# openfheorg/openfhe-development

Hardware: AMD Instinct MI355X
Metric: NTT GB/s vs HBM roofline + CKKS EvalMultKeySwitch/sec, N=2^16 L=30, 1/2/4/8 GPU (higher is better)
Workload: dtype u64; 1 GPU; batched fwd+inv negacyclic NTT, N=2^16, L=30 x 60-bit limbs, 1024 polynomials per GPU (BASELINE configs[1]); global_batch=1024, parallelism=batch-sharded x1, no data-path collective

## Files before the change

openfhe-development_amd/csrc/fhe_hip.cpp:

```cpp
#include "../../include/fhe_hip.h"

#include <algorithm>
#include <cmath>
#include <cstdio>
#include <cstdlib>
#include <map>
#include <mutex>
#include <shared_mutex>
#include <string>
#include <vector>

#include "basis_kernels.h"
#include "bfv_kernels.h"
#include "elemwise_kernels.h"
#include "host_math.h"
#include "ntt_kernels.h"
#include "ntt_static.h"
#include "ntt_row8.h"
#include "rt.h"
#include "sampler_kernels.h"
#include "blake2_kernels.h"

using namespace fhe;

static thread_local std::string g_lastError;
static fhe_status fail(fhe_status code, const std::string& msg) {
    g_lastError = msg;
    return code;
}
#define RT_CHECK(expr)                                                                  \
    do {                                                                                \
        const char* _e = (expr);                                                        \
        if (_e)                                                                         \
            return fail(FHE_ERR_DEVICE, std::string(#expr) + ": " + _e);                \
    } while (0)
#define ARG_CHECK(cond, msg)                  \
    do {                                      \
        if (!(cond))                          \
            return fail(FHE_ERR_ARG, msg);    \
    } while (0)

extern "C" const char* fhe_last_error(void) { return g_lastError.c_str(); }
extern "C" const char* fhe_version(void) {
#ifdef FHE_EMU
    return "fhe_hip 0.1 (TEST lane emulator build — not a product build)";
#else
    return "fhe_hip 0.1 (gfx950)";
#endif
}
extern "C" int fhe_device_count(void) { return rt::device_count(); }

namespace fhe {
namespace host {
bool is_prime(uint64_t n) {
    static const uint64_t w[] = {2, 3, 5, 7, 11, 13, 17, 19, 23, 29, 31, 37};
    if (n < 2)
        return false;
    for (uint64_t p : w) {
        if (n == p)
            return true;
        if (n % p == 0)
            return false;
    }
    uint64_t d = n - 1;
    int s      = 0;
    while (!(d & 1)) {
        d >>= 1;
        ++s;
    }
    for (uint64_t a : w) {
        uint64_t x = powmod(a, d, n);
        if (x == 1 || x == n - 1)
            continue;
        bool comp = true;
        for (int r = 1; r < s && comp; ++r) {
            x = mulmod(x, x, n);
            if (x == n - 1)
                comp = false;
        }
        if (comp)
            return false;
    }
    return true;
}
bool is_primitive_root_2n(uint64_t psi, uint64_t twoN, uint64_t q) {
    return psi != 0 && psi < q && powmod(psi, twoN / 2, q) == q - 1;
}
uint64_t first_prime(uint32_t bits, uint64_t m) {
    uint64_t q = (uint64_t)1 << bits, r = q % m, c = q + 1 - r;
    if (r > 0)
        c += m;
    while (!is_prime(c))
        c += m;
    return c;
}
uint64_t last_prime(uint32_t bits, uint64_t m) {
    uint64_t q = (uint64_t)1 << bits, r = q % m, c = q + 1 - r;
    if (r < 2)
        c -= m;
    while (!is_prime(c))
        c -= m;
// ... 499 lines not shown
    a.canonLevels = 1;
    while ((1u << a.canonLevels) < pp.outBound)
        ++a.canonLevels;
    if (canonOut)
        for (uint32_t i = 0; i < pp.nSteps; ++i)
            if (pp.steps[i].bHi >= pp.steps[i].bLo)
                a.canonStep = i;
    for (uint32_t i = 0; i < 6; ++i)
        a.steps[i] = i < pp.nSteps ? pp.steps[i] : NttStep{0, 0, -1, 0, 0, 0, 0, 0};
    a.sel = sel;
    const uint32_t grid        = tiles_for(c, a.rows);
    const uint32_t tilesPerRow = c->N >= (uint32_t)kTile ? (c->N >> kTileLog) : 1u;
    a.xcdSwizzle = (c->N >= (uint32_t)kTile && ((nLimbs * tilesPerRow) % 8u == 0)) ? 1u : 0u;
    a.epiMode = 0, a.epiSplit = 0, a.epiAStride = 0, a.epiAFirst = 0;
    a.epiA = nullptr, a.epiC = nullptr, a.epiOut0 = a.epiOut1 = nullptr;
    a.proMode = 0, a.proSrcLimb = 0;
    a.inDelta = 0, a.epiADelta = 0;
    return grid;
}
static int static_mode(const fhe_ctx* c, const PassPlan& pp, bool inverse) {
    const bool twoPass = c->logN > (uint32_t)kTileLog;
    const int fclass = pp.inBound <= 1 ? 1 : 9;
    return inverse ? ((pp.layoutA || !twoPass) ? 1 : 0) : fclass;
}
static bool row8_for(uint32_t T) {
    static const int forced = [] {
        const char* v = std::getenv("FHE_NTT_ROW8");
        return v && (v[0] == '0' || v[0] == '1') ? v[0] - '0' : -1;
    }();
    return forced >= 0 ? forced == 1 : T <= 11u;
}
static fhe_status launch_pass(const fhe_ctx* c, const PassPlan& pp, bool inverse, const uint64_t* xin, uint64_t* xout,
                              const LimbSel& sel, uint32_t nLimbs, uint32_t batch, bool canonOut, void* stream,
                              uint32_t inStride = 0, uint32_t inFirst = 0, uint32_t outStride = 0, uint32_t outFirst = 0,
                              const NttEpilogue* epi = nullptr, const uint32_t* proSrcLimb = nullptr, int64_t inDelta = 0) {
    NttPassArgs a;
    const uint32_t grid = fill_pass_args(c, pp, inverse, xin, xout, sel, nLimbs, batch, canonOut, inStride, inFirst, outStride,
                                         outFirst, a);
    if (inDelta) {
        if (c->logN < (uint32_t)kTileLog)
            return fail(FHE_ERR_UNSUPPORTED, "ntt: separately allocated towers need a ring of at least 4096");
        a.inDelta = inDelta;
    }
    if (proSrcLimb) {
        a.proMode = 1, a.proSrcLimb = *proSrcLimb;
        const int mode = static_mode(c, pp, inverse);
        if (pp.layoutA && !inverse && mode == 1 && pp.T == 4)
            FHE_LAUNCH_BARRIER((ntt_static_kernel<true, false, 4, 1, false, true>), grid, stream, a);
        else if (pp.layoutA && !inverse && mode == 1 && pp.T == 5)
            FHE_LAUNCH_BARRIER((ntt_static_kernel<true, false, 5, 1, false, true>), grid, stream, a);
        else
            return fail(FHE_ERR_UNSUPPORTED, "ntt: no prologue kernel for this pass shape");
        LAUNCH_CHECK();
        return FHE_OK;
    }
    if (epi && epi->mode) {
        a.epiMode = epi->mode, a.epiSplit = epi->split, a.epiAStride = epi->aStride, a.epiAFirst = epi->aFirst;
        a.epiA = epi->A, a.epiC = epi->C, a.epiOut0 = epi->out0, a.epiOut1 = epi->out1;
        a.epiADelta = epi->aDelta;
        const int mode = static_mode(c, pp, inverse);
        bool launched  = false;
#define FHE_EPI_CASE(TT, MODE) \
    if (!launched && !pp.layoutA && !inverse && pp.T == TT && mode == MODE) { \
        FHE_LAUNCH_BARRIER((ntt_static_kernel<false, false, TT, MODE, true>), grid, stream, a); \
        launched = true; \
    }
        FHE_EPI_CASE(12, 9) FHE_EPI_CASE(11, 9) FHE_EPI_CASE(10, 9) FHE_EPI_CASE(9, 9) FHE_EPI_CASE(12, 1)
#undef FHE_EPI_CASE
        if (!launched)
            return fail(FHE_ERR_UNSUPPORTED, "ntt: no epilogue kernel for this pass shape");
        LAUNCH_CHECK();
        return FHE_OK;
    }
    if (c->logN >= (uint32_t)kTileLog) {
        const int mode = static_mode(c, pp, inverse);
        bool launched  = false;
#define FHE_STATIC_CASE(LA, INV, TT, MODE) \
    if (!launched && pp.layoutA == LA && inverse == INV && pp.T == TT && mode == MODE) { \
        FHE_LAUNCH_BARRIER((ntt_static_kernel<LA, INV, TT, MODE>), grid, stream, a); \
        launched = true; \
    }
        if (!pp.layoutA && c->logN > (uint32_t)kTileLog && row8_for(pp.T)) {
            const uint32_t rgrid = a.rows << (c->logN - pp.T);
            a.xcdSwizzle         = ((nLimbs << (c->logN - pp.T)) % 8u == 0) ? 1u : 0u;
#define FHE_ROW8_CASE(INV, TT, MODE) \
    if (!launched && inverse == INV && pp.T == TT && mode == MODE) { \
        FHE_LAUNCH_BARRIER_N((r8::ntt_row8_kernel<INV, TT - 9, MODE>), rgrid, 64u << (TT - 9), stream, a); \
        launched = true; \
    }
            FHE_ROW8_CASE(false, 12, 9) FHE_ROW8_CASE(true, 12, 0) FHE_ROW8_CASE(false, 11, 9) FHE_ROW8_CASE(true, 11, 0)
            FHE_ROW8_CASE(false, 10, 9) FHE_ROW8_CASE(true, 10, 0) FHE_ROW8_CASE(false, 9, 9) FHE_ROW8_CASE(true, 9, 0)
#undef FHE_ROW8_CASE
        }
        FHE_STATIC_CASE(true, false, 4, 1) FHE_STATIC_CASE(true, true, 4, 1)
        FHE_STATIC_CASE(true, false, 5, 1) FHE_STATIC_CASE(true, true, 5, 1)
        FHE_STATIC_CASE(false, false, 12, 9) FHE_STATIC_CASE(false, true, 12, 0)
        FHE_STATIC_CASE(false, false, 11, 9) FHE_STATIC_CASE(false, true, 11, 0)
        FHE_STATIC_CASE(false, false, 10, 9) FHE_STATIC_CASE(false, true, 10, 0)
        FHE_STATIC_CASE(false, false, 9, 9) FHE_STATIC_CASE(false, true, 9, 0)
        FHE_STATIC_CASE(false, false, 12, 1) FHE_STATIC_CASE(false, true, 12, 1)
#undef FHE_STATIC_CASE
        if (!launched)
            return fail(FHE_ERR_UNSUPPORTED, "ntt: no kernel instance for this pass shape");
        LAUNCH_CHECK();
        return FHE_OK;
    }
    if (pp.layoutA) {
        if (inverse)
            FHE_LAUNCH_BARRIER((ntt_pass_kernel<true, true>), grid, stream, a);
        else
            FHE_LAUNCH_BARRIER((ntt_pass_kernel<true, false>), grid, stream, a);
    }
    else {
        if (inverse)
            FHE_LAUNCH_BARRIER((ntt_pass_kernel<false, true>), grid, stream, a);
        else
            FHE_LAUNCH_BARRIER((ntt_pass_kernel<false, false>), grid, stream, a);
    }
    LAUNCH_CHECK();
    return FHE_OK;
}

static uint32_t env_u32(const char* name, uint32_t dflt) {
    const char* v = std::getenv(name);
    return v ? (uint32_t)std::strtoul(v, nullptr, 10) : dflt;
}
static uint32_t ntt_t1(uint32_t logN) {
    const uint32_t dflt = std::max(4u, logN - (uint32_t)kTileLog);
    static const uint32_t forced = env_u32("FHE_NTT_T1", 0);
    if (forced >= 4 && forced <= 5 && logN > (uint32_t)kTileLog && logN - forced >= 9 && logN - forced <= 12)
        return forced;
    return dflt;
}

static bool ntt_epilogue_supported(const fhe_ctx* c) {
    if (c->logN < (uint32_t)kTileLog)
        return false;
    if (c->logN == (uint32_t)kTileLog)
        return true;
    const uint32_t t1 = ntt_t1(c->logN), t2 = c->logN - t1;
    return t2 == 12u || (t1 == 4u && t2 >= 9u && t2 <= 12u);
}
static bool ntt_prologue_supported(const fhe_ctx* c) {
    return c->logN > (uint32_t)kTileLog && ntt_t1(c->logN) <= 5u;
}
static fhe_status ntt_run(fhe_ctx* c, bool inverse, const uint64_t* xin, uint64_t* xout, const uint32_t* limbIdx,
                          uint32_t nLimbs, uint32_t batch, void* stream, uint32_t inStride = 0, uint32_t inFirst = 0,
                          uint32_t outStride = 0, uint32_t outFirst = 0, const NttEpilogue* epi = nullptr,
                          bool canonOut = true, const uint32_t* proSrcLimb = nullptr, int64_t inDelta = 0) {
    ARG_CHECK(c && xin && xout, "fhe_ntt: null argument");
    ARG_CHECK(batch >= 1, "fhe_ntt: batch must be >= 1");
    LimbSel sel;
    if (fhe_status s = make_sel(c, limbIdx, nLimbs, &sel, "fhe_ntt"))
        return s;
    RT_CHECK(rt::set_device(c->device));
    const uint32_t logN = c->logN;
    if (logN <= (uint32_t)kTileLog) {
        PassPlan p;
        plan_pass(inverse, false, logN, logN, &p);
        uint32_t bound = 1;
        mark_uniform(p, logN);
        if (!inverse)
            schedule_fwd(p, logN, &bound);
        p.outBound = bound;
        return launch_pass(c, p, inverse, xin, xout, sel, nLimbs, batch, canonOut, stream, inStride, inFirst, outStride, outFirst, epi,
                           nullptr, inDelta);
    }
    const uint32_t T1 = ntt_t1(logN), T2 = logN - T1;
    PassPlan pa, pb;
    plan_pass(inverse, true, logN, T1, &pa);
// ... 1065 lines not shown
    ARG_CHECK(p && devB && devA && out, "fhe_ks_key_wrap: null argument");
    fhe_ks_key* k = new fhe_ks_key;
    k->plan       = p;
    k->words      = (size_t)p->numPartQ * (p->sizeQ + p->sizeP) << p->ctx->logN;
    k->d_b        = devB;
    k->d_a        = devA;
    k->owned      = false;
    *out          = k;
    return FHE_OK;
}
extern "C" void fhe_ks_key_destroy(fhe_ks_key* k) {
    if (!k)
        return;
    if (k->owned && k->d_b)
        rt::dfree(k->d_b);
    if (k->owned && k->d_a)
        rt::dfree(k->d_a);
    delete k;
}
extern "C" uint64_t* fhe_ks_key_devptr(fhe_ks_key* k, int which) { return k ? (which ? k->d_a : k->d_b) : nullptr; }
extern "C" size_t fhe_ks_key_words(const fhe_ks_key* k) { return k ? k->words : 0; }

struct KsLayout {
    size_t coef = 0, e0 = 0, e1 = 0, md = 0, pcoef = 0, d2 = 0, k0 = 0, k1 = 0, total = 0;
    std::vector<size_t> dig;
};
static KsLayout ks_layout(const fhe_ks_plan* p, uint32_t sizeQl, uint32_t batch) {
    KsLayout w;
    const size_t N = (size_t)1 << p->ctx->logN;
    const uint32_t numParts = std::min((sizeQl + p->alpha - 1) / p->alpha, p->numPartQ);
    w.dig.assign(numParts, 0);
    size_t off = 0;
    w.coef = off, off += (size_t)batch * sizeQl * N;
    for (uint32_t j = 0; j < numParts; ++j) {
        const uint32_t start = p->alpha * j;
        const uint32_t sz    = (j == numParts - 1) ? sizeQl - start : p->alpha;
        w.dig[j] = off, off += (size_t)batch * (sizeQl - sz + p->sizeP) * N;
    }
    w.e0 = off, off += (size_t)batch * (sizeQl + p->sizeP) * N;
    w.e1 = off, off += (size_t)batch * (sizeQl + p->sizeP) * N;
    w.md = off, off += (size_t)2 * batch * sizeQl * N;
    w.pcoef = off, off += (size_t)2 * batch * p->sizeP * N;
    w.d2 = off, off += (size_t)batch * sizeQl * N;
    w.k0 = off, off += (size_t)batch * sizeQl * N;
    w.k1 = off, off += (size_t)batch * sizeQl * N;
    w.total = off;
    return w;
}
extern "C" size_t fhe_ks_workspace_bytes(const fhe_ks_plan* p, uint32_t sizeQl, uint32_t batch) {
    if (!p || sizeQl < 1 || sizeQl > p->sizeQ || batch < 1)
        return 0;
    return ks_layout(p, sizeQl, batch).total * 8;
}

static fhe_status mod_down_core(fhe_ks_plan* p, fhe_ks_plan::Level* lv, const uint64_t* x, uint32_t nTow, uint64_t* pcoef,
                                uint64_t* md, void* st, fhe_conv* down = nullptr, const NttEpilogue* epi = nullptr) {
    fhe_ctx* c            = p->ctx;
    const uint32_t sizeQl = lv->sizeQl, sizeP = p->sizeP, sizeQlP = sizeQl + sizeP;
    std::vector<uint32_t> pIdx(sizeP);
    for (uint32_t j = 0; j < sizeP; ++j)
        pIdx[j] = p->sizeQ + j;
    if (fhe_status s = ntt_run(c, true, x, pcoef, pIdx.data(), sizeP, nTow, st, sizeQlP, sizeQl))
        return s;
    if (fhe_status s = fhe_approx_switch_basis(down ? down : lv->down, pcoef, sizeP, 0, md, sizeQl, 0, nTow, st))
        return s;
    return ntt_run(c, false, md, md, nullptr, sizeQl, nTow, st, 0, 0, 0, 0, epi);
}
static fhe_status mod_down_tail(fhe_ks_plan* p, fhe_ks_plan::Level* lv, const uint64_t* x, const uint64_t* md, uint32_t nTow,
                                uint64_t* out, bool accumulate, void* st) {
    const uint32_t sizeQl = lv->sizeQl, sizeQlP = sizeQl + p->sizeP;
    if (accumulate)
        return elem_run<OP_SUB_MUL_CONST_ACC>(p->ctx, out, x, md, lv->d_PInv, nullptr, sizeQl, nTow, st, "fhe_approx_mod_down",
                                              sizeQlP, 0);
    return elem_run<OP_SUB_MUL_CONST>(p->ctx, out, x, md, lv->d_PInv, nullptr, sizeQl, nTow, st, "fhe_approx_mod_down", sizeQlP, 0);
}
static fhe_status mod_down_run(fhe_ks_plan* p, fhe_ks_plan::Level* lv, const uint64_t* x, uint32_t nTow, uint64_t* out,
                               uint64_t* pcoef, uint64_t* md, void* st) {
    if (fhe_status s = mod_down_core(p, lv, x, nTow, pcoef, md, st))
        return s;
    return mod_down_tail(p, lv, x, md, nTow, out, false, st);
}

static fhe_status ks_precompute_run(fhe_ks_plan* p, fhe_ks_plan::Level* lv, const uint64_t* cin, uint32_t batch,
                                    uint64_t* ws, const KsLayout& w, void* st) {
    fhe_ctx* c            = p->ctx;
    const uint32_t sizeQl = lv->sizeQl;
    if (fhe_status s = fhe_ntt_inv_oop(c, cin, ws + w.coef, nullptr, sizeQl, batch, st))
        return s;
    for (uint32_t j = 0; j < lv->numParts; ++j) {
        const uint32_t nc = (uint32_t)lv->cidx[j].size();
        uint64_t* dj      = ws + w.dig[j];
        if (fhe_status s = fhe_approx_switch_basis(lv->up[j], ws + w.coef, sizeQl, p->alpha * j, dj, nc, 0, batch, st))
            return s;
        if (fhe_status s = ntt_run(c, false, dj, dj, lv->cidx[j].data(), nc, batch, st, 0, 0, 0, 0, nullptr, false))
            return s;
    }
    return FHE_OK;
}
static fhe_status ks_inner_multi_launch(fhe_ks_plan* p, fhe_ks_plan::Level* lv, const fhe_ks_key* const* keys, uint32_t nKeys,
                                        const uint64_t* cin, uint32_t batch, uint64_t* const* e0, uint64_t* const* e1,
                                        const uint64_t* first, const TwPair* dP, uint64_t* ws, const KsLayout& w, void* st,
                                        uint32_t towOff = 0) {
    fhe_ctx* c            = p->ctx;
    const uint32_t sizeQl = lv->sizeQl, sizeP = p->sizeP, sizeQlP = sizeQl + sizeP;
    const uint32_t tilesPerRow = c->N >= (uint32_t)kTile ? (c->N >> kTileLog) : 1u;
    for (uint32_t t0 = 0; t0 < nKeys; t0 += (uint32_t)kMaxMultiKeys) {
        KsInnerMultiArgs g;
        const uint32_t nt = std::min<uint32_t>(kMaxMultiKeys, nKeys - t0);
        for (uint32_t j = 0; j < (uint32_t)kMaxDigits; ++j) {
            g.nc[j]     = j < lv->numParts ? (uint32_t)lv->cidx[j].size() : 0u;
            g.digits[j] = j < lv->numParts ? ws + w.dig[j] + (((size_t)towOff * g.nc[j]) << c->logN) : nullptr;
        }
        for (uint32_t t = 0; t < (uint32_t)kMaxMultiKeys; ++t) {
            const uint32_t tt = t < nt ? t0 + t : t0;
            g.keyB[t] = keys[tt]->d_b, g.keyA[t] = keys[tt]->d_a, g.out0[t] = e0[tt], g.out1[t] = e1[tt];
        }
        g.c = cin + (((size_t)towOff * sizeQl) << c->logN), g.first = first, g.firstC = dP;
        g.lc = c->d_lc, g.mu128 = c->d_mu128, g.red = c->d_red;
        g.logN = c->logN, g.batch = batch, g.sizeQl = sizeQl, g.sizeQ = p->sizeQ, g.sizeP = sizeP;
        g.numDigits = lv->numParts, g.alpha = p->alpha, g.nKeys = nt;
        const uint64_t grid = (((uint64_t)tilesPerRow * sizeQlP + 7) / 8) * 8 * batch;
        static const uint32_t ksm = env_u32("FHE_KSM", 1);
        uintptr_t bits = (uintptr_t)g.c | (uintptr_t)g.first;
        for (uint32_t j = 0; j < lv->numParts && j < (uint32_t)kMaxDigits; ++j)
            bits |= (uintptr_t)g.digits[j];
        for (uint32_t t = 0; t < nt; ++t)
            bits |= (uintptr_t)g.keyB[t] | (uintptr_t)g.keyA[t] | (uintptr_t)g.out0[t] | (uintptr_t)g.out1[t];
        const bool wide = (bits & 15u) == 0 && c->N >= 2;
        if (lv->numParts <= 3 && ksm == 1 && wide)
            FHE_LAUNCH((ks_inner_multi_kernel<3, 2, true>), grid, st, g);
        else if (lv->numParts <= 3 && ksm == 2 && wide)
            FHE_LAUNCH((ks_inner_multi_kernel<3, 2, false>), grid, st, g);
        else if (lv->numParts <= 3 && ksm == 3)
            FHE_LAUNCH((ks_inner_multi_kernel<3, 1, false>), grid, st, g);
        else if (lv->numParts <= 3)
            FHE_LAUNCH((ks_inner_multi_kernel<3>), grid, st, g);
        else if (lv->numParts <= 4)
            FHE_LAUNCH((ks_inner_multi_kernel<4>), grid, st, g);
        else
            FHE_LAUNCH((ks_inner_multi_kernel<8>), grid, st, g);
        LAUNCH_CHECK();
    }
    return FHE_OK;
}
static fhe_status ks_inner_run(fhe_ks_plan* p, fhe_ks_plan::Level* lv, const fhe_ks_key* key, const uint64_t* cin,
                               uint32_t batch, uint64_t* e0, uint64_t* e1, uint64_t* ws, const KsLayout& w, void* st,
                               uint32_t towOff = 0) {
    fhe_ctx* c            = p->ctx;
    const uint32_t sizeQl = lv->sizeQl, sizeP = p->sizeP, sizeQlP = sizeQl + sizeP;
    const uint32_t tilesPerRow = c->N >= (uint32_t)kTile ? (c->N >> kTileLog) : 1u;
    if (lv->numParts <= (uint32_t)kMaxDigits)
        return ks_inner_multi_launch(p, lv, &key, 1, cin, batch, &e0, &e1, nullptr, nullptr, ws, w, st, towOff);
    for (uint32_t j0 = 0; j0 < lv->numParts; j0 += (uint32_t)kMaxDigits) {
        KsInnerArgs g;
        const uint32_t nd = std::min<uint32_t>(kMaxDigits, lv->numParts - j0);
        for (uint32_t j = 0; j < (uint32_t)kMaxDigits; ++j) {
            g.nc[j]     = j < nd ? (uint32_t)lv->cidx[j0 + j].size() : 0u;
            g.digits[j] = j < nd ? ws + w.dig[j0 + j] + (((size_t)towOff * g.nc[j]) << c->logN) : nullptr;
        }
        g.c = cin + (((size_t)towOff * sizeQl) << c->logN), g.keyB = key->d_b, g.keyA = key->d_a;
        g.out0 = e0, g.out1 = e1;
        g.lc = c->d_lc, g.mu128 = c->d_mu128, g.red = c->d_red;
        g.logN = c->logN, g.batch = batch, g.sizeQl = sizeQl, g.sizeQ = p->sizeQ, g.sizeP = sizeP;
        g.numDigits = nd, g.alpha = p->alpha, g.j0 = j0, g.acc = j0 > 0;
        FHE_LAUNCH(ks_inner_product_kernel, (((uint64_t)tilesPerRow * sizeQlP + 7) / 8) * 8 * batch, st, g);
        LAUNCH_CHECK();
    }
    return FHE_OK;
}
static fhe_status ks_inner_multi_run(fhe_ks_plan* p, fhe_ks_plan::Level* lv, const fhe_ks_key* const* keys, uint32_t nKeys,
                                     const uint64_t* cin, uint32_t batch, uint64_t* const* e0, uint64_t* const* e1,
                                     const uint64_t* first, const TwPair* dP, uint64_t* ws, const KsLayout& w, void* st) {
    if (lv->numParts <= (uint32_t)kMaxDigits)
        return ks_inner_multi_launch(p, lv, keys, nKeys, cin, batch, e0, e1, first, dP, ws, w, st);
    const uint32_t sizeQl = lv->sizeQl, sizeQlP = sizeQl + p->sizeP;
    for (uint32_t t = 0; t < nKeys; ++t) {
        if (fhe_status s = ks_inner_run(p, lv, keys[t], cin, batch, e0[t], e1[t], ws, w, st))
            return s;
        if (first)
            if (fhe_status s = elem_run<OP_MUL_CONST_ADD>(p->ctx, e0[t], first, e0[t], dP, nullptr, sizeQl, batch, st,
                                                          "fhe_eval_fast_rotation_ext", 0, 0, sizeQlP, 0, sizeQlP, 0))
                return s;
    }
    return FHE_OK;
}
extern "C" fhe_status fhe_inner_product(fhe_ctx* c, uint32_t nTerms, const uint64_t* const* x, const uint64_t* const* k0,
                                        const uint64_t* const* k1, const uint32_t* keyRow, const uint32_t* limbIdx,
                                        uint32_t rows, uint32_t batch, uint64_t* out0, uint64_t* out1, void* st) {
    ARG_CHECK(c && x && k0 && out0, "fhe_inner_product: null argument");
    ARG_CHECK((k1 != nullptr) == (out1 != nullptr), "fhe_inner_product: the second key and the second output go together");
    ARG_CHECK(batch >= 1, "fhe_inner_product: batch must be >= 1");
    ARG_CHECK(nTerms >= 1, "fhe_inner_product: no terms");
    InnerRowsArgs g;
    if (fhe_status s = make_sel(c, limbIdx, rows, &g.sel, "fhe_inner_product"))
        return s;
    for (uint32_t i = 0; i < (uint32_t)kMaxLimbs; ++i) {
        const uint32_t kr = i < rows ? (keyRow ? keyRow[i] : i) : 0u;
        ARG_CHECK(kr < 256u, "fhe_inner_product: key row out of range");
        g.keyRow[i] = (uint8_t)kr;
    }
    for (uint32_t j = 0; j < nTerms; ++j)
        ARG_CHECK(x[j] && k0[j] && (!k1 || k1[j]), "fhe_inner_product: null term");
    RT_CHECK(rt::set_device(c->device));
    g.out0 = out0, g.out1 = out1, g.lc = c->d_lc, g.mu128 = c->d_mu128;
    g.logN = c->logN, g.batch = batch, g.rows = rows;
    const uint32_t tilesPerRow = c->N >= (uint32_t)kTile ? (c->N >> kTileLog) : 1u;
    for (uint32_t t0 = 0; t0 < nTerms; t0 += (uint32_t)kMaxDigits) {
        const uint32_t nt = std::min<uint32_t>(kMaxDigits, nTerms - t0);
        for (uint32_t j = 0; j < (uint32_t)kMaxDigits; ++j) {
            g.x[j]  = j < nt ? x[t0 + j] : nullptr;
            g.k0[j] = j < nt ? k0[t0 + j] : nullptr;
            g.k1[j] = (j < nt && k1) ? k1[t0 + j] : nullptr;
        }
        g.nTerms = nt, g.acc = t0 > 0;
        FHE_LAUNCH(inner_rows_kernel, (uint64_t)tilesPerRow * rows * batch, st, g);
        LAUNCH_CHECK();
    }
    return FHE_OK;
}
static fhe_status ks_fast_run(fhe_ks_plan* p, fhe_ks_plan::Level* lv, const fhe_ks_key* key, const uint64_t* cin,
                              uint32_t batch, uint64_t* out0, uint64_t* out1, uint64_t* ws, const KsLayout& w, void* st,
                              bool accumulate) {
    fhe_ctx* c            = p->ctx;
    const uint32_t sizeQl = lv->sizeQl;
    if (fhe_status s = ks_inner_run(p, lv, key, cin, batch, ws + w.e0, ws + w.e1, ws, w, st))
        return s;
    if (ntt_epilogue_supported(c)) {
        NttEpilogue epi;
        epi.mode = accumulate ? 2u : 1u, epi.split = batch, epi.aStride = sizeQl + p->sizeP, epi.aFirst = 0;
        epi.A = ws + w.e0, epi.C = lv->d_PInv, epi.out0 = out0, epi.out1 = out1;
        return mod_down_core(p, lv, ws + w.e0, 2 * batch, ws + w.pcoef, ws + w.md, st, nullptr, &epi);
    }
    if (fhe_status s = mod_down_core(p, lv, ws + w.e0, 2 * batch, ws + w.pcoef, ws + w.md, st))
        return s;
    if (fhe_status s = mod_down_tail(p, lv, ws + w.e0, ws + w.md, batch, out0, accumulate, st))
        return s;
    return mod_down_tail(p, lv, ws + w.e1, ws + w.md + ((size_t)batch * sizeQl << c->logN), batch, out1, accumulate, st);
}
static fhe_status keyswitch_run(fhe_ks_plan* p, const fhe_ks_key* key, const uint64_t* cin, uint32_t sizeQl,
                                uint32_t batch, uint64_t* out0, uint64_t* out1, uint64_t* ws, const KsLayout& w,
                                void* st, bool accumulate = false) {
    fhe_ks_plan::Level* lv = nullptr;
    if (fhe_status s = ks_level(p, sizeQl, &lv))
        return s;
    if (fhe_status s = ks_precompute_run(p, lv, cin, batch, ws, w, st))
        return s;
    return ks_fast_run(p, lv, key, cin, batch, out0, out1, ws, w, st, accumulate);
}

extern "C" fhe_status fhe_keyswitch_hybrid(fhe_ks_plan* p, const fhe_ks_key* key, const uint64_t* cin, uint32_t sizeQl,
                                           uint32_t batch, uint64_t* out0, uint64_t* out1, void* ws, size_t wsBytes,
                                           void* st) {
    ARG_CHECK(p && key && cin && out0 && out1 && ws, "fhe_keyswitch_hybrid: null argument");
    ARG_CHECK(key->plan == p, "fhe_keyswitch_hybrid: key belongs to another plan");
    ARG_CHECK(sizeQl >= 1 && sizeQl <= p->sizeQ && batch >= 1, "fhe_keyswitch_hybrid: bad level or batch");
    const KsLayout w = ks_layout(p, sizeQl, batch);
    ARG_CHECK(wsBytes >= w.total * 8, "fhe_keyswitch_hybrid: workspace too small");
    RT_CHECK(rt::set_device(p->ctx->device));
    return keyswitch_run(p, key, cin, sizeQl, batch, out0, out1, (uint64_t*)ws, w, st);
}

extern "C" fhe_status fhe_keyswitch_hybrid_acc(fhe_ks_plan* p, const fhe_ks_key* key, const uint64_t* cin, uint32_t sizeQl,
                                               uint32_t batch, uint64_t* acc0, uint64_t* acc1, void* ws, size_t wsBytes, void* st) {
    ARG_CHECK(p && key && cin && acc0 && acc1 && ws, "fhe_keyswitch_hybrid_acc: null argument");
    ARG_CHECK(key->plan == p, "fhe_keyswitch_hybrid_acc: key belongs to another plan");
    ARG_CHECK(sizeQl >= 1 && sizeQl <= p->sizeQ && batch >= 1, "fhe_keyswitch_hybrid_acc: bad level or batch");
    const KsLayout w = ks_layout(p, sizeQl, batch);
    ARG_CHECK(wsBytes >= w.total * 8, "fhe_keyswitch_hybrid_acc: workspace too small");
    RT_CHECK(rt::set_device(p->ctx->device));
    return keyswitch_run(p, key, cin, sizeQl, batch, acc0, acc1, (uint64_t*)ws, w, st, true);
}

extern "C" fhe_status fhe_ckks_eval_mult(fhe_ks_plan* p, const fhe_ks_key* key, const uint64_t* a0, const uint64_t* a1,
                                         const uint64_t* b0, const uint64_t* b1, uint32_t sizeQl, uint32_t batch,
                                         uint64_t* c0, uint64_t* c1, void* wsv, size_t wsBytes, void* st) {
    ARG_CHECK(p && key && a0 && a1 && b0 && b1 && c0 && c1 && wsv, "fhe_ckks_eval_mult: null argument");
    ARG_CHECK(key->plan == p, "fhe_ckks_eval_mult: key belongs to another plan");
    ARG_CHECK(sizeQl >= 1 && sizeQl <= p->sizeQ && batch >= 1, "fhe_ckks_eval_mult: bad level or batch");
    const KsLayout w = ks_layout(p, sizeQl, batch);
    ARG_CHECK(wsBytes >= w.total * 8, "fhe_ckks_eval_mult: workspace too small");
    fhe_ctx* c   = p->ctx;
    uint64_t* ws = (uint64_t*)wsv;
    RT_CHECK(rt::set_device(c->device));
    if (fhe_status s = fhe_tensor(c, a0, a1, b0, b1, c0, c1, ws + w.d2, nullptr, sizeQl, batch, st))
        return s;
    return keyswitch_run(p, key, ws + w.d2, sizeQl, batch, c0, c1, ws, w, st, true);
}

#define KS_COMMON_CHECKS(who)                                                                              \
    ARG_CHECK(p && ws, who ": null argument");                                                             \
    ARG_CHECK(sizeQl >= 1 && sizeQl <= p->sizeQ && batch >= 1, who ": bad level or batch");                \
    const KsLayout w = ks_layout(p, sizeQl, batch);                                                        \
    ARG_CHECK(wsBytes >= w.total * 8, who ": workspace too small");                                        \
    RT_CHECK(rt::set_device(p->ctx->device));                                                              \
    fhe_ks_plan::Level* lv = nullptr;                                                                      \
    if (fhe_status s_ = ks_level(p, sizeQl, &lv))                                                          \
        return s_;

extern "C" fhe_status fhe_ks_precompute(fhe_ks_plan* p, const uint64_t* c1, uint32_t sizeQl, uint32_t batch, void* ws,
                                        size_t wsBytes, void* st) {
    KS_COMMON_CHECKS("fhe_ks_precompute")
    ARG_CHECK(c1, "fhe_ks_precompute: null argument");
    return ks_precompute_run(p, lv, c1, batch, (uint64_t*)ws, w, st);
}
extern "C" fhe_status fhe_ks_fast_keyswitch(fhe_ks_plan* p, const fhe_ks_key* key, const uint64_t* c1, uint32_t sizeQl,
                                            uint32_t batch, uint64_t* out0, uint64_t* out1, void* ws, size_t wsBytes,
                                            void* st) {
    KS_COMMON_CHECKS("fhe_ks_fast_keyswitch")
    ARG_CHECK(key && c1 && out0 && out1 && key->plan == p, "fhe_ks_fast_keyswitch: bad key or null argument");
    return ks_fast_run(p, lv, key, c1, batch, out0, out1, (uint64_t*)ws, w, st, false);
}
extern "C" fhe_status fhe_eval_fast_rotation(fhe_ks_plan* p, const fhe_ks_key* key, const uint64_t* c0, const uint64_t* c1,
                                             uint32_t k, uint32_t sizeQl, uint32_t batch, uint64_t* out0, uint64_t* out1,
                                             void* ws, size_t wsBytes, void* st) {
    KS_COMMON_CHECKS("fhe_eval_fast_rotation")
    ARG_CHECK(key && c0 && c1 && out0 && out1 && key->plan == p, "fhe_eval_fast_rotation: bad key or null argument");
    ARG_CHECK(k % 2 == 1, "Automorphism index not odd");
    uint64_t* wsp = (uint64_t*)ws;
    fhe_ctx* c    = p->ctx;
    if (fhe_status s = ks_fast_run(p, lv, key, c1, batch, wsp + w.k0, wsp + w.k1, wsp, w, st, false))
        return s;
    if (fhe_status s = fhe_add(c, wsp + w.k0, wsp + w.k0, c0, nullptr, sizeQl, batch, st))
        return s;
    if (fhe_status s = fhe_automorph(c, out0, wsp + w.k0, k, 1, nullptr, sizeQl, batch, st))
        return s;
    return fhe_automorph(c, out1, wsp + w.k1, k, 1, nullptr, sizeQl, batch, st);
}
extern "C" fhe_status fhe_eval_automorphism(fhe_ks_plan* p, const fhe_ks_key* key, const uint64_t* c0, const uint64_t* c1,
                                            uint32_t k, uint32_t sizeQl, uint32_t batch, uint64_t* out0, uint64_t* out1,
                                            void* ws, size_t wsBytes, void* st) {
// ... 1196 lines not shown
```

Measured before the change: 2281 GB/s.

## Fuse second NTT pass of key-switch digits into the inner-product kernel

Result: no change. 2280 GB/s (-0.1%).

```diff
diff --git a/openfhe-development_amd/csrc/fhe_hip.cpp b/openfhe-development_amd/csrc/fhe_hip.cpp
--- a/openfhe-development_amd/csrc/fhe_hip.cpp
+++ b/openfhe-development_amd/csrc/fhe_hip.cpp
@@ -17,6 +17,7 @@
 #include "ntt_kernels.h"
 #include "ntt_static.h"
 #include "ntt_row8.h"
+#include "ks_row8.h"
 #include "rt.h"
 #include "sampler_kernels.h"
 #include "blake2_kernels.h"
@@ -682,10 +683,11 @@
     }
         if (!pp.layoutA && c->logN > (uint32_t)kTileLog && row8_for(pp.T)) {
             const uint32_t rgrid = a.rows << (c->logN - pp.T);
-            a.xcdSwizzle         = ((nLimbs << (c->logN - pp.T)) % 8u == 0) ? 1u : 0u;
+            NttPassArgs a8       = a;
+            a8.xcdSwizzle        = ((nLimbs << (c->logN - pp.T)) % 8u == 0) ? 1u : 0u;
 #define FHE_ROW8_CASE(INV, TT, MODE) \
     if (!launched && inverse == INV && pp.T == TT && mode == MODE) { \
-        FHE_LAUNCH_BARRIER_N((r8::ntt_row8_kernel<INV, TT - 9, MODE>), rgrid, 64u << (TT - 9), stream, a); \
+        FHE_LAUNCH_BARRIER_N((r8::ntt_row8_kernel<INV, TT - 9, MODE>), rgrid, 64u << (TT - 9), stream, a8); \
         launched = true; \
     }
             FHE_ROW8_CASE(false, 12, 9) FHE_ROW8_CASE(true, 12, 0) FHE_ROW8_CASE(false, 11, 9) FHE_ROW8_CASE(true, 11, 0)
@@ -1917,7 +1919,7 @@
 }
 
 static fhe_status ks_precompute_run(fhe_ks_plan* p, fhe_ks_plan::Level* lv, const uint64_t* cin, uint32_t batch,
-                                    uint64_t* ws, const KsLayout& w, void* st) {
+                                    uint64_t* ws, const KsLayout& w, void* st, bool fused = false) {
     fhe_ctx* c            = p->ctx;
     const uint32_t sizeQl = lv->sizeQl;
     if (fhe_status s = fhe_ntt_inv_oop(c, cin, ws + w.coef, nullptr, sizeQl, batch, st))
@@ -1927,6 +1929,19 @@
         uint64_t* dj      = ws + w.dig[j];
         if (fhe_status s = fhe_approx_switch_basis(lv->up[j], ws + w.coef, sizeQl, p->alpha * j, dj, nc, 0, batch, st))
             return s;
+        if (fused) {
+            LimbSel sel;
+            if (fhe_status s = make_sel(c, lv->cidx[j].data(), nc, &sel, "fhe_keyswitch_hybrid"))
+                return s;
+            PassPlan pa;
+            plan_pass(false, true, c->logN, ntt_t1(c->logN), &pa);
+            mark_uniform(pa, c->logN);
+            uint32_t bound = 1;
+            schedule_fwd(pa, c->logN, &bound);
+            if (fhe_status s = launch_pass(c, pa, false, dj, dj, sel, nc, batch, false, st))
+                return s;
+            continue;
+        }
         if (fhe_status s = ntt_run(c, false, dj, dj, lv->cidx[j].data(), nc, batch, st, 0, 0, 0, 0, nullptr, false))
             return s;
     }
@@ -2053,12 +2068,60 @@
     }
     return FHE_OK;
 }
+static bool ks_fused_for(const fhe_ks_plan* p, const fhe_ks_plan::Level* lv) {
+    static const int forced = [] {
+        const char* v = std::getenv("FHE_KS_FUSED");
+        return v && (v[0] == '0' || v[0] == '1') ? v[0] - '0' : -1;
+    }();
+    const fhe_ctx* c = p->ctx;
+    if (forced == 0 || c->logN <= (uint32_t)kTileLog || lv->numParts > (uint32_t)kMaxDigits)
+        return false;
+    const uint32_t t2 = c->logN - ntt_t1(c->logN);
+    return t2 >= 9u && t2 <= 12u;
+}
+static fhe_status ks_fused_inner_run(fhe_ks_plan* p, fhe_ks_plan::Level* lv, const fhe_ks_key* key, const uint64_t* cin,
+                                     uint32_t batch, uint64_t* e0, uint64_t* e1, uint64_t* ws, const KsLayout& w, void* st) {
+    fhe_ctx* c            = p->ctx;
+    const uint32_t sizeQl = lv->sizeQl, sizeQlP = sizeQl + p->sizeP;
+    const uint32_t T      = c->logN - ntt_t1(c->logN);
+    r8::KsRow8Args g;
+    uintptr_t bits = (uintptr_t)cin | (uintptr_t)key->d_b | (uintptr_t)key->d_a | (uintptr_t)e0 | (uintptr_t)e1;
+    for (uint32_t j = 0; j < (uint32_t)kMaxDigits; ++j) {
+        g.nc[j]     = j < lv->numParts ? (uint32_t)lv->cidx[j].size() : 0u;
+        g.digits[j] = j < lv->numParts ? ws + w.dig[j] : nullptr;
+    }
+    if (bits & 15u)
+        return fail(FHE_ERR_UNSUPPORTED, "key switch: the fused inner product needs 16-byte aligned towers");
+    g.c = cin, g.keyB = key->d_b, g.keyA = key->d_a, g.out0 = e0, g.out1 = e1;
+    g.tw = c->d_tw, g.q = c->d_q, g.red = c->d_red, g.mu128 = c->d_mu128;
+    g.logN = c->logN, g.batch = batch, g.sizeQl = sizeQl, g.sizeQ = p->sizeQ, g.sizeP = p->sizeP;
+    g.numDigits = lv->numParts, g.alpha = p->alpha;
+    g.xcdSwizzle = ((sizeQlP << (c->logN - T)) % 8u == 0) ? 1u : 0u;
+    const uint64_t grid = ((uint64_t)batch * sizeQlP) << (c->logN - T);
+    static const uint32_t stx = env_u32("FHE_KS_FUSED_STORE", 0);
+    bool launched = false;
+#define FHE_KSR8_CASE(TT) \
+    if (!launched && T == TT) { \
+        if (stx) \
+            FHE_LAUNCH_BARRIER_N((r8::ks_row8_inner_kernel<TT - 9, true>), grid, 64u << (TT - 9), st, g); \
+        else \
+            FHE_LAUNCH_BARRIER_N((r8::ks_row8_inner_kernel<TT - 9, false>), grid, 64u << (TT - 9), st, g); \
+        launched = true; \
+    }
+    FHE_KSR8_CASE(9) FHE_KSR8_CASE(10) FHE_KSR8_CASE(11) FHE_KSR8_CASE(12)
+#undef FHE_KSR8_CASE
+    if (!launched)
+        return fail(FHE_ERR_UNSUPPORTED, "key switch: no fused inner-product kernel for this ring");
+    LAUNCH_CHECK();
+    return FHE_OK;
+}
 static fhe_status ks_fast_run(fhe_ks_plan* p, fhe_ks_plan::Level* lv, const fhe_ks_key* key, const uint64_t* cin,
                               uint32_t batch, uint64_t* out0, uint64_t* out1, uint64_t* ws, const KsLayout& w, void* st,
-                              bool accumulate) {
+                              bool accumulate, bool fused = false) {
     fhe_ctx* c            = p->ctx;
     const uint32_t sizeQl = lv->sizeQl;
-    if (fhe_status s = ks_inner_run(p, lv, key, cin, batch, ws + w.e0, ws + w.e1, ws, w, st))
+    if (fhe_status s = fused ? ks_fused_inner_run(p, lv, key, cin, batch, ws + w.e0, ws + w.e1, ws, w, st)
+                             : ks_inner_run(p, lv, key, cin, batch, ws + w.e0, ws + w.e1, ws, w, st))
         return s;
     if (ntt_epilogue_supported(c)) {
         NttEpilogue epi;
@@ -2078,9 +2141,10 @@
     fhe_ks_plan::Level* lv = nullptr;
     if (fhe_status s = ks_level(p, sizeQl, &lv))
         return s;
-    if (fhe_status s = ks_precompute_run(p, lv, cin, batch, ws, w, st))
-        return s;
-    return ks_fast_run(p, lv, key, cin, batch, out0, out1, ws, w, st, accumulate);
+    const bool fused = ks_fused_for(p, lv) && (((uintptr_t)cin | (uintptr_t)ws | (uintptr_t)key->d_b | (uintptr_t)key->d_a) & 15u) == 0;
+    if (fhe_status s = ks_precompute_run(p, lv, cin, batch, ws, w, st, fused))
+        return s;
+    return ks_fast_run(p, lv, key, cin, batch, out0, out1, ws, w, st, accumulate, fused);
 }
 
 extern "C" fhe_status fhe_keyswitch_hybrid(fhe_ks_plan* p, const fhe_ks_key* key, const uint64_t* cin, uint32_t sizeQl,
diff --git a/openfhe-development_amd/csrc/ks_row8.h b/openfhe-development_amd/csrc/ks_row8.h
--- /dev/null
+++ b/openfhe-development_amd/csrc/ks_row8.h
@@ -0,0 +1,289 @@
+#ifndef FHE_KS_ROW8_H
+#define FHE_KS_ROW8_H
+#include "basis_kernels.h"
+#include "ntt_row8.h"
+
+namespace fhe {
+namespace r8 {
+
+struct KsRow8Args {
+    const uint64_t* c;
+    const uint64_t* digits[kMaxDigits];
+    const uint64_t* keyB;
+    const uint64_t* keyA;
+    uint64_t* out0;
+    uint64_t* out1;
+    const TwPair* tw;
+    const uint64_t* q;
+    const uint64_t* red;
+    const uint64_t* mu128;
+    uint32_t logN, batch, sizeQl, sizeQ, sizeP, numDigits, alpha, xcdSwizzle;
+    uint32_t nc[kMaxDigits];
+};
+
+FHE_HD void mac128(u128w& acc, uint64_t a, uint64_t b) {
+    const uint32_t al = (uint32_t)a, ah = (uint32_t)(a >> 32), bl = (uint32_t)b, bh = (uint32_t)(b >> 32);
+    const uint64_t p0 = mul32x32(al, bl);
+    const uint64_t p1 = mad64(al, bh, p0 >> 32);
+    const uint64_t p2 = mad64(ah, bl, (uint32_t)p1);
+    const uint64_t hi = mad64(ah, bh, p1 >> 32) + (p2 >> 32);
+    const uint64_t lo = (p0 & 0xffffffffull) | (p2 << 32);
+    acc.lo += lo;
+    acc.hi += hi + (acc.lo < lo);
+}
+
+#if defined(__HIP_DEVICE_COMPILE__) && defined(FHE_PINNED_ASM)
+#define FHE_KSR8_MAC2(X0, X1, X2, X3, Y0, Y1, Y2, Y3)                                                              \
+    asm volatile(                                                                                                  \
+        "v_mad_u64_u32 v[" #X0 ":" #X1 "], s[40:41], %[al], %[xl], v[" #X0 ":" #X1 "]\n\t"                         \
+        "v_mad_u64_u32 v[" #Y0 ":" #Y1 "], s[46:47], %[al], %[yl], v[" #Y0 ":" #Y1 "]\n\t"                         \
+        "v_mad_u64_u32 v[36:37], vcc, %[al], %[xh], 0\n\t"                                                         \
+        "v_mad_u64_u32 v[38:39], vcc, %[al], %[yh], 0\n\t"                                                         \
+        "v_mad_u64_u32 v[36:37], s[42:43], %[ah], %[xl], v[36:37]\n\t"                                             \
+        "v_mad_u64_u32 v[38:39], s[48:49], %[ah], %[yl], v[38:39]\n\t"                                             \
+        "v_mad_u64_u32 v[" #X2 ":" #X3 "], vcc, %[ah], %[xh], v[" #X2 ":" #X3 "]\n\t"                              \
+        "v_mad_u64_u32 v[" #Y2 ":" #Y3 "], vcc, %[ah], %[yh], v[" #Y2 ":" #Y3 "]\n\t"                              \
+        "v_add_co_u32_e64 v" #X1 ", s[44:45], v" #X1 ", v36\n\t"                                                   \
+        "v_add_co_u32_e64 v" #Y1 ", s[50:51], v" #Y1 ", v38\n\t"                                                   \
+        "v_addc_co_u32_e64 v" #X2 ", s[40:41], v" #X2 ", 0, s[40:41]\n\t"                                          \
+        "v_addc_co_u32_e64 v" #Y2 ", s[46:47], v" #Y2 ", 0, s[46:47]\n\t"                                          \
+        "v_addc_co_u32_e64 v" #X3 ", vcc, v" #X3 ", 0, s[42:43]\n\t"                                               \
+        "v_addc_co_u32_e64 v" #Y3 ", vcc, v" #Y3 ", 0, s[48:49]\n\t"                                               \
+        "v_addc_co_u32_e64 v" #X2 ", s[44:45], v" #X2 ", v37, s[44:45]\n\t"                                        \
+        "v_addc_co_u32_e64 v" #Y2 ", s[50:51], v" #Y2 ", v39, s[50:51]\n\t"                                        \
+        "v_addc_co_u32_e64 v" #X3 ", vcc, v" #X3 ", 0, s[40:41]\n\t"                                               \
+        "v_addc_co_u32_e64 v" #Y3 ", vcc, v" #Y3 ", 0, s[46:47]\n\t"                                               \
+        "v_addc_co_u32_e64 v" #X3 ", vcc, v" #X3 ", 0, s[44:45]\n\t"                                               \
+        "v_addc_co_u32_e64 v" #Y3 ", vcc, v" #Y3 ", 0, s[50:51]\n\t"                                               \
+        : "+{v[" #X0 ":" #X1 "]}"(x.lo), "+{v[" #X2 ":" #X3 "]}"(x.hi), "+{v[" #Y0 ":" #Y1 "]}"(y.lo), "+{v[" #Y2 ":" #Y3 "]}"(y.hi) \
+        : [al] "v"(al), [ah] "v"(ah), [xl] "v"(xl), [xh] "v"(xh), [yl] "v"(yl), [yh] "v"(yh)                       \
+        : "v36", "v37", "v38", "v39", "vcc", "s40", "s41", "s42", "s43", "s44", "s45", "s46", "s47", "s48", "s49", "s50", "s51")
+template <int K>
+__device__ __forceinline__ void mac2(u128w& x, u128w& y, uint64_t a, uint64_t bx, uint64_t by) {
+    const uint32_t al = (uint32_t)a, ah = (uint32_t)(a >> 32);
+    const uint32_t xl = (uint32_t)bx, xh = (uint32_t)(bx >> 32), yl = (uint32_t)by, yh = (uint32_t)(by >> 32);
+    if constexpr (K == 0) FHE_KSR8_MAC2(64, 65, 66, 67, 96, 97, 98, 99);
+    if constexpr (K == 1) FHE_KSR8_MAC2(68, 69, 70, 71, 100, 101, 102, 103);
+    if constexpr (K == 2) FHE_KSR8_MAC2(72, 73, 74, 75, 104, 105, 106, 107);
+    if constexpr (K == 3) FHE_KSR8_MAC2(76, 77, 78, 79, 108, 109, 110, 111);
+    if constexpr (K == 4) FHE_KSR8_MAC2(80, 81, 82, 83, 112, 113, 114, 115);
+    if constexpr (K == 5) FHE_KSR8_MAC2(84, 85, 86, 87, 116, 117, 118, 119);
+    if constexpr (K == 6) FHE_KSR8_MAC2(88, 89, 90, 91, 120, 121, 122, 123);
+    if constexpr (K == 7) FHE_KSR8_MAC2(92, 93, 94, 95, 124, 125, 126, 127);
+}
+#undef FHE_KSR8_MAC2
+#else
+template <int K>
+FHE_HD void mac2(u128w& x, u128w& y, uint64_t a, uint64_t bx, uint64_t by) {
+    mac128(x, a, bx);
+    mac128(y, a, by);
+}
+#endif
+
+struct Red128 {
+    uint64_t q, c64, c64p, muhi;
+};
+FHE_HD Red128 red128_make(uint64_t q, uint64_t mulo, uint64_t muhi) { return Red128{q, 0 - muhi * q, mulo, muhi}; }
+FHE_HD uint64_t red128(const u128w s, const Red128 k) {
+    const uint64_t t = s.hi * k.c64 - mulhi64(s.hi, k.c64p) * k.q;
+    const uint64_t u = s.lo - mulhi64(s.lo, k.muhi) * k.q;
+    FHE_BOUND_CHECK(t < (k.q << 1) && u < (k.q << 1), "ks_row8: a partial reduction of 2q or more");
+    return csub(csub(t + u, k.q << 1), k.q);
+}
+
+#if defined(__HIP_DEVICE_COMPILE__)
+#define FHE_KSR8_OPAQUE_V(x) asm volatile("" : "+v"(x))
+#else
+#define FHE_KSR8_OPAQUE_V(x) ((void)0)
+#endif
+#define FHE_KSR8_LANE()               \
+    uint32_t tq_ = t;                 \
+    FHE_KSR8_OPAQUE_V(tq_);           \
+    const uint32_t l = tq_ & 63u, lhi = l >> 3, llo = l & 7u; \
+    (void)lhi, (void)llo
+
+template <int WB>
+FHE_DEV void fwd_row_to_m(uint64_t (&r)[8], const uint64_t* src, uint64_t* lds, uint64_t* reg, const TwPair* tw, uint32_t t, uint32_t wv,
+                          uint32_t tr, uint32_t jbase, uint32_t logN, const BflyConst c) {
+    constexpr uint32_t threads = 64u << WB;
+    constexpr int WLOW         = 3 - WB;
+    using S = FwdSched<WB, 2>;
+    auto x1 = [](int rr) { return (uint32_t)kRegion * ((uint32_t)rr >> WLOW) + (64u << WB) * ((uint32_t)rr & ((1u << WLOW) - 1u)); };
+    if constexpr (WB > 0) {
+        {
+            FHE_KSR8_LANE();
+            const uint64_t* s0 = src + tq_;
+#pragma unroll
+            for (int k = 0; k < 8; ++k)
+                r[k] = FHE_GLD(&s0[threads * (uint32_t)k]);
+        }
+        fwd_step<true, WB, S::sweep(0)>(r, tw, tr, 6 + WB, logN, c, S::sweep(0) ? 2u : (uint32_t)S::before(0));
+        FHE_KSR8_LANE();
+        uint64_t* Lw = lds + tq_;
+#pragma unroll
+        for (int k = 0; k < 8; ++k)
+            FHE_LDS_ST(Lw[x1(k)], r[k]);
+        FHE_SSYNC();
+        const uint64_t* Lr = reg + l;
+#pragma unroll
+        for (int k = 0; k < 8; ++k)
+            FHE_LDS_LD(r[k], Lr[64 * k]);
+    }
+    else {
+        FHE_KSR8_LANE();
+        const uint64_t* s0 = src + l;
+#pragma unroll
+        for (int k = 0; k < 8; ++k)
+            r[k] = FHE_GLD(&s0[64u * (uint32_t)k]);
+    }
+    fwd_step<true, 3, S::sweep(1)>(r, tw, (jbase >> 9) + wv, 6, logN, c, S::sweep(1) ? 2u : (uint32_t)S::before(1));
+    {
+        FHE_KSR8_LANE();
+        FHE_WAVE_SYNC();
+        uint64_t* Lw = reg + l;
+#pragma unroll
+        for (int k = 0; k < 8; ++k)
+            FHE_LDS_ST(Lw[72 * k], r[k]);
+        FHE_WAVE_SYNC();
+        const uint64_t* Lr = reg + 72u * lhi + llo;
+#pragma unroll
+        for (int k = 0; k < 8; ++k)
+            FHE_LDS_LD(r[k], Lr[8 * k]);
+        fwd_step<false, 3, S::sweep(2)>(r, tw, (jbase >> 6) + (wv << 3) + lhi, 3, logN, c, S::sweep(2) ? 2u : (uint32_t)S::before(2));
+    }
+    {
+        FHE_KSR8_LANE();
+        FHE_WAVE_SYNC();
+        uint64_t* Lw = reg + fc3(lhi) + llo;
+#pragma unroll
+        for (int k = 0; k < 8; ++k)
+            FHE_LDS_ST(Lw[33 * k], r[k]);
+        FHE_WAVE_SYNC();
+        const uint64_t* Lr = reg + fc3(lhi) + 33u * llo;
+#pragma unroll
+        for (int k = 0; k < 8; ++k)
+            FHE_LDS_LD(r[k], Lr[k]);
+        fwd_step<false, 3, S::sweep(3)>(r, tw, (jbase >> 3) + (wv << 6) + l, 0, logN, c, S::sweep(3) ? 2u : (uint32_t)S::before(3));
+    }
+}
+
+template <int WB, bool STX>
+FHE_DEV void ks_row8_inner_core(const KsRow8Args& g, uint64_t* lds) {
+    static_assert(WB >= 0 && WB <= 3, "ks_row8: 1, 2, 4 or 8 waves per tile");
+    constexpr uint32_t tileLog = 9u + (uint32_t)WB;
+    const uint32_t t       = FHE_TID;
+    const uint32_t wv      = WB ? FHE_UNIFORM(t >> 6) : 0u;
+    const uint32_t logN    = g.logN;
+    const uint32_t trLog   = logN - tileLog;
+    const uint32_t sizeQlP = g.sizeQl + g.sizeP;
+    uint64_t* reg = lds + (size_t)wv * kRegion;
+    uint32_t tile = FHE_BID;
+    if (g.xcdSwizzle) {
+        const uint32_t xcd = tile & 7u, s = tile >> 3;
+        const uint32_t bb = s % g.batch, pair = (s / g.batch) * 8u + xcd;
+        tile = ((bb * sizeQlP + (pair >> trLog)) << trLog) + (pair & ((1u << trLog) - 1u));
+    }
+    const uint32_t row = tile >> trLog, tr = tile & ((1u << trLog) - 1u);
+    const uint32_t b = row / sizeQlP, i = row % sizeQlP;
+    const uint32_t jbase = tr << tileLog;
+    const uint32_t idx   = FHE_UNIFORM(i < g.sizeQl ? i : i + (g.sizeQ - g.sizeQl));
+    const uint64_t q     = FHE_ULOAD64(g.q, idx);
+    const uint64_t twoq = q << 1, nq = 0 - q;
+    const TwPair* tw    = g.tw + ((uint64_t)idx << logN);
+    const uint64_t redc = FHE_ULOAD64(g.red, idx);
+    const BflyConst c{(uint32_t)nq, (uint32_t)(nq >> 32), q, twoq, 0 - twoq, twoq + q, (uint32_t)redc, (uint32_t)(redc >> 32)};
+
+    u128w acc0[8], acc1[8];
+#pragma unroll
+    for (int k = 0; k < 8; ++k)
+        acc0[k] = acc1[k] = u128w{0, 0};
+    bool transformed = false;
+    for (uint32_t j = 0; j < g.numDigits; ++j) {
+        const uint32_t start = j * g.alpha;
+        const uint32_t sz    = sizeQlP - g.nc[j];
+        const bool own       = i >= start && i < start + sz;
+        uint64_t r[8];
+        if (own) {
+            FHE_KSR8_LANE();
+            const uint64_t* s0 = g.c + (((uint64_t)b * g.sizeQl + i) << logN) + jbase + (wv << 9) + 8u * l;
+#pragma unroll
+            for (int k = 0; k < 8; k += 2) {
+                const U64x2 v = *reinterpret_cast<const U64x2*>(s0 + k);
+                r[k] = v.a, r[k + 1] = v.b;
+            }
+        }
+        else {
+            const uint32_t pos = i < start ? i : i - sz;
+            const uint64_t* src = g.digits[j] + (((uint64_t)b * g.nc[j] + pos) << logN) + jbase;
+            if (WB > 0 && transformed)
+                FHE_SSYNC();
+            fwd_row_to_m<WB>(r, src, lds, reg, tw, t, wv, tr, jbase, logN, c);
+            transformed = true;
+        }
+        {
+            FHE_KSR8_LANE();
+            const uint64_t koff = (((uint64_t)j * (g.sizeQ + g.sizeP) + idx) << logN) + jbase + (wv << 9) + 8u * l;
+            const uint64_t* kB = g.keyB + koff;
+            const uint64_t* kA = g.keyA + koff;
+            U64x2 vb[4], va[4];
+#pragma unroll
+            for (int k = 0; k < 4; ++k) {
+                vb[k] = *reinterpret_cast<const U64x2*>(kB + 2 * k);
+                va[k] = *reinterpret_cast<const U64x2*>(kA + 2 * k);
+            }
+#define FHE_KSR8_PAIR(K)                                                               \
+    mac2<K>(acc0[K], acc1[K], r[K], vb[K / 2].a, va[K / 2].a);                         \
+    mac2<K + 1>(acc0[K + 1], acc1[K + 1], r[K + 1], vb[K / 2].b, va[K / 2].b);
+            FHE_KSR8_PAIR(0) FHE_KSR8_PAIR(2) FHE_KSR8_PAIR(4) FHE_KSR8_PAIR(6)
+#undef FHE_KSR8_PAIR
+        }
+    }
+    const Red128 rk = red128_make(q, FHE_ULOAD64(g.mu128, 2 * idx), FHE_ULOAD64(g.mu128, 2 * idx + 1));
+    const uint64_t orow = (((uint64_t)b * sizeQlP + i) << logN) + jbase + (wv << 9);
+    if constexpr (!STX) {
+        FHE_KSR8_LANE();
+        uint64_t* d0 = g.out0 + orow + 8u * l;
+        uint64_t* d1 = g.out1 + orow + 8u * l;
+#pragma unroll
+        for (int k = 0; k < 8; k += 2) {
+            *reinterpret_cast<U64x2*>(d0 + k) = U64x2{red128(acc0[k], rk), red128(acc0[k + 1], rk)};
+            *reinterpret_cast<U64x2*>(d1 + k) = U64x2{red128(acc1[k], rk), red128(acc1[k + 1], rk)};
+        }
+    }
+    else {
+#pragma unroll
+        for (int e = 0; e < 2; ++e) {
+            uint64_t v[8];
+#pragma unroll
+            for (int k = 0; k < 8; ++k)
+                v[k] = red128(e ? acc1[k] : acc0[k], rk);
+            FHE_KSR8_LANE();
+            FHE_WAVE_SYNC();
+            uint64_t* Lw = reg + fc4(lhi) + llo;
+#pragma unroll
+            for (int k = 0; k < 8; ++k)
+                FHE_LDS_ST(Lw[36 * k], v[k]);
+            FHE_WAVE_SYNC();
+            const uint64_t* Lr = reg + lhi + 36u * llo;
+#pragma unroll
+            for (int k = 0; k < 8; ++k)
+                FHE_LDS_LD(v[k], Lr[fc4((uint32_t)k)]);
+            uint64_t* d0 = (e ? g.out1 : g.out0) + orow + l;
+#pragma unroll
+            for (int k = 0; k < 8; ++k)
+                FHE_GST(&d0[64u * (uint32_t)k], v[k]);
+        }
+    }
+}
+#undef FHE_KSR8_LANE
+#undef FHE_KSR8_OPAQUE_V
+
+template <int WB, bool STX>
+FHE_GLOBAL void FHE_LAUNCH_BOUNDS2(64 << WB, 4) ks_row8_inner_kernel(const KsRow8Args g) {
+    FHE_SHARED_U64(lds, (1 << WB) * kRegion);
+    ks_row8_inner_core<WB, STX>(g, lds);
+}
+
+}
+}
+#endif
```
